# EnterpriseCV-6/Season-NeRF

Hardware: AMD Instinct MI355X
Metric: ray-samples/sec (4096 rays x 96 samples forward render, T_NeRF 8x256) (higher is better)
Workload: dtype i8x3 (16-bit fixed point as two int8 digits on v_mfma_i32_32x32x32_i8, exact int32 accumulate, fp32 epilogue)

## Files before the change

### include/season_nerf_hip.h

```cpp
#ifndef SEASON_NERF_HIP_H
#define SEASON_NERF_HIP_H

#include <stddef.h>
#include <stdint.h>

#ifdef __cplusplus
extern "C" {
#endif

#define SNERF_OK 0
#define SNERF_E_INVALID (-1)
#define SNERF_E_MISSING (-2)
#define SNERF_E_HIP (-3)
#define SNERF_E_STATE (-4)

typedef struct snerf_model snerf_model;

const char* snerf_last_error(void);
int snerf_abi_version(void);

snerf_model* snerf_model_create(int layer_width, int n_classes);
int snerf_model_set_tensor(snerf_model* m, const char* key, const float* host_data, size_t numel);
int snerf_model_finalize(snerf_model* m);
void snerf_model_destroy(snerf_model* m);
int snerf_model_width(const snerf_model* m);
int snerf_model_classes(const snerf_model* m);

#define SNERF_PREC_BF16X3 0
#define SNERF_PREC_BF16 1
#define SNERF_PREC_I8X3 2
#define SNERF_PREC_AUTO 3
int snerf_model_set_precision(snerf_model* m, int precision);
int snerf_model_precision(const snerf_model* m);

typedef struct snerf_i8_estimate {
    double head_rms[4];
    double hidden_rms;
    double worst;
    double rgb_pred;
    double budget;
    int64_t acc_bound;
    int ok;
} snerf_i8_estimate;
int snerf_model_i8_estimate(snerf_model* m, snerf_i8_estimate* out);
int snerf_model_resolve_precision(snerf_model* m);

int snerf_model_pack_host(snerf_model* m, int program, uint8_t* stream_out, size_t* stream_bytes,
                          float* bias_out, size_t* bias_floats);

int snerf_group_forward(const snerf_model* m, int64_t n_groups, const float* d_time, const float* d_sun,
                        float* d_classes, float* d_sky_raw, float* d_sky, void* stream);

typedef struct snerf_field_out {
    float* d_rho;
    float* d_solar_vis;
    float* d_col_raw;
    float* d_adjust;
    float* d_col;
    float* d_adjust_col;
    float* d_points;
} snerf_field_out;

int snerf_field_forward_points(const snerf_model* m, int variant, int64_t n_points, const float* d_points,
                               int64_t group_size, const float* d_sun, const float* d_classes,
                               const snerf_field_out* out, void* stream);

int snerf_field_forward_rays(const snerf_model* m, int variant, int64_t n_rays, int n_samples,
                             const float* d_top, const float* d_bot, const float* d_tvals,
                             int64_t rays_per_group, const float* d_sun, const float* d_classes,
                             const snerf_field_out* out, void* stream);

int snerf_field_ray_visibility(const snerf_model* m, int64_t n_rays, int n_samples, const float* d_top, const float* d_bot,
                               const float* d_tvals, int flags, float* d_vis, void* stream);

typedef struct snerf_composite_out {
    float* d_rgb;
    float* d_albedo;
    float* d_pv;
    float* d_pe;
    float* d_ps;
    float* d_delta;
    float* d_shadow;
    float* d_acc;
    float* d_surf_loc;
    float* d_surf_dist;
} snerf_composite_out;

int snerf_composite_rays(int64_t n_rays, int n_samples, const float* d_top, const float* d_bot, const float* d_tvals,
                         const float* d_rho, const float* d_col, const float* d_solar_vis, const float* d_sky,
                         int flags, const float* d_rho_prior, float trust,
                         const snerf_composite_out* out, void* stream);
int snerf_composite_rays_dt(int64_t n_rays, int n_samples, const float* d_top, const float* d_bot, const float* d_tvals,
                            const float* d_rho, const float* d_col, const float* d_solar_vis, const float* d_sky,
                            int flags, const float* d_rho_prior, const float* d_trust,
                            const snerf_composite_out* out, void* stream);

size_t snerf_render_workspace_bytes(int64_t n_rays, int n_samples, int n_classes);
int snerf_render_rays(const snerf_model* m, int64_t n_rays, int n_samples, const float* d_top, const float* d_bot,
                      const float* d_tvals, const float* d_sun, const float* d_time, int flags,
                      float* d_rgb, const snerf_field_out* field_out, const snerf_composite_out* comp_out,
                      void* d_workspace, size_t workspace_bytes, void* stream);

typedef struct snerf_sweep_out {
    float* d_season;
    float* d_shaded;
    float* d_base;
    float* d_shadow_adjust;
    float* d_raw_shadow;
    float* d_classic;
} snerf_sweep_out;

int snerf_composite_sweep(int64_t n_rays, int n_samples, int n_classes, int n_times, const float* d_top,
                          const float* d_bot, const float* d_tvals, const float* d_deltas, const float* d_rho, const float* d_col_raw,
                          const float* d_adjust, const float* d_solar_vis, const float* d_sky, const float* d_class_vecs,
                          int flags, const snerf_sweep_out* out, void* stream);

typedef struct snerf_trainer snerf_trainer;
snerf_trainer* snerf_trainer_create(int layer_width, int n_classes);
void snerf_trainer_destroy(snerf_trainer* t);
int snerf_trainer_classes(const snerf_trainer* t);
int64_t snerf_trainer_param_floats(const snerf_trainer* t);
int64_t snerf_trainer_buffer_floats(const snerf_trainer* t);
int snerf_trainer_tensor_count(const snerf_trainer* t);
int snerf_trainer_tensor_info(const snerf_trainer* t, int index, char* key, int key_cap, int* is_buffer, int64_t* offset,
                              int64_t* numel, int* rows, int* cols);
size_t snerf_trainer_workspace_bytes(snerf_trainer* t, int64_t n_rays, int64_t n_solar_rays, int n_samples);
int snerf_trainer_bind(snerf_trainer* t, float* d_params, float* d_grads, float* d_adam_m, float* d_adam_v, float* d_buffers,
                       void* d_workspace, size_t workspace_bytes, int64_t n_rays, int64_t n_solar_rays, int n_samples);
int snerf_trainer_bound_sizes(const snerf_trainer* t, int64_t* n_rays, int64_t* n_solar_rays, int* n_samples);
int snerf_trainer_forward_image(snerf_trainer* t, int64_t n_rays, int n_samples, const float* d_top, const float* d_bot,
                                const float* d_tvals, const float* d_sun, const float* d_time, int train_bn, int flags,
                                const snerf_composite_out* out, float* d_sky, float* d_classes,
                                const snerf_field_out* per_sample, void* stream);
int snerf_trainer_backward_image(snerf_trainer* t, const float* d_g_rgb, const float* d_g_albedo, const float* d_g_sky,
// ... 60 lines not shown
```

### season_nerf_amd/_lib.py

```python
import ctypes as C
import os

HERE = os.path.dirname(os.path.abspath(__file__))
LIB_PATH = os.environ.get("SNERF_LIB", os.path.join(HERE, "libseason_nerf_hip.so"))

_f = C.POINTER(C.c_float)


class FieldOut(C.Structure):
    _fields_ = [(n, C.c_void_p) for n in
                ("d_rho", "d_solar_vis", "d_col_raw", "d_adjust", "d_col", "d_adjust_col", "d_points")]


class CompositeOut(C.Structure):
    _fields_ = [(n, C.c_void_p) for n in
                ("d_rgb", "d_albedo", "d_pv", "d_pe", "d_ps", "d_delta", "d_shadow", "d_acc", "d_surf_loc", "d_surf_dist")]


class SweepOut(C.Structure):
    _fields_ = [(n, C.c_void_p) for n in ("d_season", "d_shaded", "d_base", "d_shadow_adjust", "d_raw_shadow", "d_classic")]


class I8Estimate(C.Structure):
    _fields_ = [("head_rms", C.c_double * 4), ("hidden_rms", C.c_double), ("worst", C.c_double),
                ("rgb_pred", C.c_double), ("budget", C.c_double), ("acc_bound", C.c_int64), ("ok", C.c_int)]


ALLREDUCE_FN = C.CFUNCTYPE(C.c_int, C.c_void_p, C.c_void_p, C.c_int64, C.c_int, C.c_void_p)

_lib = None


def lib():
    global _lib
    if _lib is not None:
        return _lib
    if not os.path.exists(LIB_PATH):
        raise RuntimeError(
            f"season_nerf_amd: HIP library not built ({LIB_PATH} missing). Run `python season_nerf_amd/build.py` "
            "(needs hipcc, gfx950). There is no CPU fallback.")
    L = C.CDLL(LIB_PATH)
    vp, i64, i32 = C.c_void_p, C.c_int64, C.c_int
    L.snerf_last_error.restype = C.c_char_p
    L.snerf_abi_version.restype = i32
    L.snerf_model_create.restype = vp
    L.snerf_model_create.argtypes = [i32, i32]
    L.snerf_model_set_tensor.argtypes = [vp, C.c_char_p, vp, C.c_size_t]
    L.snerf_model_finalize.argtypes = [vp]
    L.snerf_model_destroy.argtypes = [vp]
    L.snerf_model_destroy.restype = None
    L.snerf_model_width.argtypes = [vp]
    L.snerf_model_classes.argtypes = [vp]
    L.snerf_model_set_precision.argtypes = [vp, i32]
    L.snerf_model_precision.argtypes = [vp]
    L.snerf_model_i8_estimate.argtypes = [vp, C.POINTER(I8Estimate)]
    L.snerf_model_resolve_precision.argtypes = [vp]
    L.snerf_model_pack_host.argtypes = [vp, i32, vp, C.POINTER(C.c_size_t), vp, C.POINTER(C.c_size_t)]
    L.snerf_group_forward.argtypes = [vp, i64, vp, vp, vp, vp, vp, vp]
    L.snerf_field_forward_points.argtypes = [vp, i32, i64, vp, i64, vp, vp, C.POINTER(FieldOut), vp]
    L.snerf_field_forward_rays.argtypes = [vp, i32, i64, i32, vp, vp, vp, i64, vp, vp, C.POINTER(FieldOut), vp]
    L.snerf_field_ray_visibility.argtypes = [vp, i64, i32, vp, vp, vp, i32, vp, vp]
    L.snerf_composite_rays.argtypes = [i64, i32, vp, vp, vp, vp, vp, vp, vp, i32, vp, C.c_float,
                                       C.POINTER(CompositeOut), vp]
    L.snerf_composite_rays_dt.argtypes = [i64, i32, vp, vp, vp, vp, vp, vp, vp, i32, vp, vp, C.POINTER(CompositeOut), vp]
    L.snerf_render_workspace_bytes.restype = C.c_size_t
    L.snerf_render_workspace_bytes.argtypes = [i64, i32, i32]
    L.snerf_render_rays.argtypes = [vp, i64, i32, vp, vp, vp, vp, vp, i32, vp, C.POINTER(FieldOut),
                                    C.POINTER(CompositeOut), vp, C.c_size_t, vp]
    L.snerf_composite_sweep.argtypes = [i64, i32, i32, i32, vp, vp, vp, vp, vp, vp, vp, vp, vp, vp, i32, C.POINTER(SweepOut), vp]
    f32p = vp
    L.snerf_trainer_create.restype = vp
    L.snerf_trainer_create.argtypes = [i32, i32]
    L.snerf_trainer_destroy.argtypes = [vp]
    L.snerf_trainer_destroy.restype = None
    L.snerf_trainer_bound_sizes.restype = i32
    L.snerf_trainer_bound_sizes.argtypes = [vp, vp, vp, vp]
    L.snerf_trainer_classes.restype = i32
    L.snerf_trainer_classes.argtypes = [vp]
    L.snerf_trainer_param_floats.restype = i64
    L.snerf_trainer_param_floats.argtypes = [vp]
    L.snerf_trainer_buffer_floats.restype = i64
    L.snerf_trainer_buffer_floats.argtypes = [vp]
    L.snerf_trainer_tensor_count.argtypes = [vp]
    L.snerf_trainer_tensor_info.argtypes = [vp, i32, C.c_char_p, i32, C.POINTER(i32), C.POINTER(i64), C.POINTER(i64),
                                            C.POINTER(i32), C.POINTER(i32)]
    L.snerf_trainer_workspace_bytes.restype = C.c_size_t
    L.snerf_trainer_workspace_bytes.argtypes = [vp, i64, i64, i32]
    L.snerf_trainer_bind.argtypes = [vp, f32p, f32p, f32p, f32p, f32p, vp, C.c_size_t, i64, i64, i32]
    L.snerf_trainer_forward_image.argtypes = [vp, i64, i32, vp, vp, vp, vp, vp, i32, i32, C.POINTER(CompositeOut), vp, vp,
                                              C.POINTER(FieldOut), vp]
    L.snerf_trainer_backward_image.argtypes = [vp, vp, vp, vp, vp, vp, C.c_float, vp, vp, vp]
    L.snerf_trainer_backward_image_dt.argtypes = [vp, vp, vp, vp, vp, vp, vp, vp, vp, vp]
    L.snerf_trainer_backward_points.argtypes = [vp, vp, vp, vp, vp, vp, vp]
    L.snerf_trainer_forward_solar.argtypes = [vp, i64, i32, vp, vp, vp, vp, i32, vp, vp, vp, vp, vp, vp, vp, vp]
    L.snerf_trainer_backward_solar.argtypes = [vp, vp, vp]
    L.snerf_trainer_zero_grad.argtypes = [vp, vp]
    L.snerf_trainer_set_allreduce.argtypes = [vp, vp, vp, i32]
    L.snerf_trainer_debug_read.argtypes = [vp, C.c_char_p, vp, i64]
    L.snerf_trainer_adam_step.argtypes = [vp, C.c_float, C.c_float, C.c_float, C.c_float, i32, vp]
    L.snerf_trainer_adam_step_dev.argtypes = [vp, vp, vp]
    L.snerf_adam_step.argtypes = [vp, vp, vp, vp, i64, C.c_float, C.c_float, C.c_float, C.c_float, i32, vp]
    L.snerf_rays_from_camera.argtypes = [vp, i32, i32, i32, vp, vp, vp]
    L.snerf_ray_grid.argtypes = [i32, i32, i32, i64, i64, vp, i32, vp, vp, vp, vp, vp]
    L.snerf_prior_density.argtypes = [i64, vp, vp, vp, i32, i32, vp, vp, vp]
    L.snerf_surface_distance.argtypes = [i64, i32, vp, vp, vp, vp, i32, i32, vp, vp, vp]
    L.snerf_image_error.argtypes = [i64, vp, vp, vp, vp]
    L.snerf_transmittance.argtypes = [i64, i32, vp, vp, vp, vp]
    L.snerf_linear_scratch_bytes.restype = C.c_size_t
    L.snerf_linear_scratch_bytes.argtypes = [i32, i32]
    L.snerf_linear_forward.argtypes = [i64, i32, i32, vp, i64, vp, vp, C.c_float, vp, i64, vp, i32, vp, C.c_size_t, vp, i32, vp]
    L.snerf_linear_dgrad.argtypes = [i64, i32, i32, vp, i64, vp, i32, C.c_float, i32, vp, i64, i32, vp, C.c_size_t, vp, i64, vp, vp, vp, vp, vp]
    L.snerf_linear_wgrad.argtypes = [i64, i32, i32, vp, i64, vp, i64, C.c_float, vp, i32, vp, i32, vp]
    L.snerf_field_kernel_info.argtypes = [vp, i64, C.POINTER(i32), C.POINTER(i32), C.POINTER(i32)]
    _lib = L
    return L


PRECISIONS = {"bf16x3": 0, "bf16": 1, "i8x3": 2, "auto": 3}
PRECISION_NAMES = {0: "bf16x3", 1: "bf16", 2: "i8x3"}


def check(rc, what):
    if rc != 0:
        raise RuntimeError(f"season_nerf_amd: {what} failed (code {rc}): {lib().snerf_last_error().decode()}")


EXPORTS = ["snerf_last_error", "snerf_abi_version", "snerf_model_create", "snerf_model_set_tensor",
           "snerf_model_finalize", "snerf_model_destroy", "snerf_model_width", "snerf_model_classes",
           "snerf_model_set_precision", "snerf_model_precision", "snerf_model_i8_estimate", "snerf_model_resolve_precision",
           "snerf_model_pack_host", "snerf_group_forward", "snerf_field_forward_points", "snerf_field_forward_rays", "snerf_field_ray_visibility",
           "snerf_composite_rays", "snerf_composite_rays_dt", "snerf_composite_sweep", "snerf_render_workspace_bytes", "snerf_render_rays", "snerf_rays_from_camera", "snerf_ray_grid", "snerf_field_kernel_info",
           "snerf_prior_density", "snerf_surface_distance", "snerf_image_error", "snerf_transmittance",
           "snerf_linear_scratch_bytes", "snerf_linear_forward", "snerf_linear_dgrad", "snerf_linear_wgrad",
           "snerf_trainer_create", "snerf_trainer_destroy", "snerf_trainer_classes", "snerf_trainer_param_floats", "snerf_trainer_buffer_floats",
           "snerf_trainer_tensor_count", "snerf_trainer_tensor_info", "snerf_trainer_workspace_bytes", "snerf_trainer_bind", "snerf_trainer_bound_sizes",
           "snerf_trainer_forward_image", "snerf_trainer_backward_image", "snerf_trainer_backward_image_dt", "snerf_trainer_backward_points", "snerf_trainer_forward_solar",
           "snerf_trainer_backward_solar", "snerf_trainer_zero_grad", "snerf_trainer_set_allreduce", "snerf_trainer_adam_step", "snerf_trainer_adam_step_dev", "snerf_adam_step", "snerf_trainer_debug_read",
           "snerf_loss_scratch_bytes", "snerf_loss_scratch_init", "snerf_loss_terms_forward", "snerf_loss_terms_backward"]
```

### season_nerf_amd/build.py

```python
import os
import subprocess
import sys
from concurrent.futures import ThreadPoolExecutor

HERE = os.path.dirname(os.path.abspath(__file__))
REPO = os.path.dirname(HERE)
CSRC = os.path.join(HERE, "csrc")
OBJ = os.path.join(REPO, "build", "obj")
LIB = os.path.join(HERE, "libseason_nerf_hip.so")
SOURCES = ["kernels.hip", "kernels_i8.hip", "kernels_i8x2.hip", "kernels_i8_w512.hip", "kernels_ks.hip", "api.cpp", "pack.cpp", "gemm.hip", "gemm16.hip", "gemm_areg.hip", "train_kernels.hip", "train.cpp", "dsm.hip"]
HEADERS = ["gemm_common.h", "gemm_rows.h", "kernels.h", "linear_product.h", "mlp_device.h", "mlp_bf16_device.h", "mlp_i8_device.h", "pack.h", "program.h", "train.h", os.path.join("..", "..", "include", "season_nerf_hip.h")]
FLAGS = ["-std=c++17", "-O3", "--offload-arch=gfx950", "-fPIC", "-ffp-contract=off",
         "-mllvm", "-amdgpu-mfma-vgpr-form=1",
         "-Wno-unused-command-line-argument"]


EXTRA = {"kernels_i8_w512.hip": ["-mllvm", "-pragma-unroll-threshold=1000000"],
         "kernels_ks.hip": ["-mllvm", "-pragma-unroll-threshold=1000000"],
         "gemm_areg.hip": ["-mllvm", "-pragma-unroll-threshold=1000000"]}
INCLUDED = {"kernels_i8_w512.hip": ["kernels_i8.hip"]}


def _hipcc():
    return os.environ.get("HIPCC", "/opt/rocm/bin/hipcc")


def _newest_header():
    return max(os.path.getmtime(os.path.join(CSRC, h)) for h in HEADERS if os.path.exists(os.path.join(CSRC, h)))


def _obj(src):
    return os.path.join(OBJ, src + ".o")


def _deps(src):
    d = _obj(src) + ".d"
    if not os.path.exists(d):
        return None
    txt = open(d).read().replace("\\\n", " ")
    return [f for f in txt.split(":", 1)[1].split() if f.startswith(REPO)] if ":" in txt else None


def _stale(src, hdr_t):
    o = _obj(src)
    if not os.path.exists(o):
        return True
    t = os.path.getmtime(o)
    deps = _deps(src)
    if deps is not None:
        return any((not os.path.exists(f)) or os.path.getmtime(f) > t for f in deps)
    return any(os.path.getmtime(os.path.join(CSRC, f)) > t for f in [src] + INCLUDED.get(src, [])) or hdr_t > t


def needs_build():
    if not os.path.exists(LIB):
        return True
    hdr_t = _newest_header()
    t = os.path.getmtime(LIB)
    return any(os.path.getmtime(os.path.join(CSRC, s)) > t for s in SOURCES) or hdr_t > t


def _compile(src, verbose):
    cmd = [_hipcc()] + FLAGS + EXTRA.get(src, []) + ["-MD", "-MF", _obj(src) + ".d", "-c", os.path.join(CSRC, src), "-o", _obj(src)]
    if verbose:
        print(" ".join(cmd), flush=True)
    subprocess.check_call(cmd)


def build(force=False, verbose=True, jobs=None):
    if not force and not needs_build():
        return LIB
    os.makedirs(OBJ, exist_ok=True)
    hdr_t = _newest_header()
    todo = [s for s in SOURCES if force or _stale(s, hdr_t)]
    jobs = jobs or min(len(todo) or 1, max(1, (os.cpu_count() or 2) - 1), 6)
    with ThreadPoolExecutor(max_workers=jobs) as ex:
        list(ex.map(lambda s: _compile(s, verbose), todo))
    cmd = [_hipcc(), "--offload-arch=gfx950", "-shared", "-fPIC", "-o", LIB] + [_obj(s) for s in SOURCES]
    if verbose:
        print(" ".join(cmd), flush=True)
    subprocess.check_call(cmd)
    return LIB


OPS_LIB = os.path.join(HERE, "libseason_nerf_ops.so")
OPS_SRC = os.path.join(CSRC, "ops.cpp")


def build_ops(force=False, verbose=True):
    import torch
    if not force and os.path.exists(OPS_LIB) and os.path.getmtime(OPS_LIB) > max(os.path.getmtime(OPS_SRC), os.path.getmtime(LIB),
                                                                                  os.path.getmtime(os.path.join(REPO, "include", "season_nerf_hip.h"))):
        return OPS_LIB
# ... 18 lines not shown
```

### season_nerf_amd/csrc/api.cpp

```cpp
#include "../../include/season_nerf_hip.h"

#include <hip/hip_runtime.h>

#include <cstdio>
#include <cstdlib>
#include <cmath>
#include <cstring>
#include <string>

#include "kernels.h"
#include "pack.h"
#include "train.h"

#ifndef SNERF_I8_BUDGET
#define SNERF_I8_BUDGET 1.0e-4
#endif

using namespace snerf;

static thread_local std::string g_err;
static int fail(int code, const std::string& msg) {
    g_err = msg;
    return code;
}
int snerf_set_error(int code, const std::string& msg) { return fail(code, msg); }
static int fail_hip(hipError_t e, const char* what) {
    return fail(SNERF_E_HIP, std::string(what) + ": " + hipGetErrorString(e));
}

struct snerf_model {
    int W = 0, C = 0;
    int precision = SNERF_PREC_BF16X3;
    bool auto_mode = false;
    bool resolved = true;
    bool have_estimate = false;
    snerf_i8_estimate estimate{};
    Weights w;
    bool finalized = false;
    Packed host[2];
    Packed host_i8;
    Packed host_ks;
    Packed host_ksg;
    float* d_group_f32 = nullptr;
    size_t g32_off[10] = {0};
    uint8_t* d_stream[2] = {nullptr, nullptr};
    float* d_bias[2] = {nullptr, nullptr};
    uint8_t* d_stream_i8 = nullptr;
    float* d_table_i8 = nullptr;
    uint8_t* d_stream_ks = nullptr;
    float* d_bias_ks = nullptr;
    uint8_t* d_stream_ksg = nullptr;
    float* d_bias_ksg = nullptr;
    int n_cu = 0;
};

extern "C" {

const char* snerf_last_error(void) { return g_err.c_str(); }
int snerf_abi_version(void) { return 8; }

snerf_model* snerf_model_create(int layer_width, int n_classes) {
    if (layer_width != 64 && layer_width != 256 && layer_width != 512) {
        fail(SNERF_E_INVALID, "layer_width " + std::to_string(layer_width) +
                                  " has no compiled kernel (built widths: 64, 256, 512)");
        return nullptr;
    }
    if (n_classes < 1 || n_classes > kMaxClasses) {
        fail(SNERF_E_INVALID, "n_classes must be in [1," + std::to_string(kMaxClasses) + "]");
        return nullptr;
    }
    snerf_model* m = new snerf_model();
    m->W = layer_width;
    m->C = n_classes;
    return m;
}

int snerf_model_set_precision(snerf_model* m, int precision) {
    if (!m) return fail(SNERF_E_INVALID, "NULL model");
    if (m->finalized) return fail(SNERF_E_STATE, "model already finalized (set the precision before snerf_model_finalize)");
    if (precision != SNERF_PREC_BF16X3 && precision != SNERF_PREC_BF16 && precision != SNERF_PREC_I8X3 && precision != SNERF_PREC_AUTO)
        return fail(SNERF_E_INVALID, "unknown precision mode " + std::to_string(precision));
    m->auto_mode = precision == SNERF_PREC_AUTO;
    m->resolved = !m->auto_mode;
    m->precision = precision;
    return SNERF_OK;
}
// ... 173 lines not shown
                m->g32_off[2 * i + j] = blob.size();
                blob.insert(blob.end(), t->data.begin(), t->data.end());
                blob.resize((blob.size() + 3) / 4 * 4, 0.f);
            }
        const int W = m->W, C = m->C, W4 = W / 4;
        const size_t want[10] = {(size_t)W * 10, (size_t)W, (size_t)W * W, (size_t)W, (size_t)C * W, (size_t)C, (size_t)W4 * 27, (size_t)W4, (size_t)3 * W4, 3};
        for (int i = 0; i < 10; ++i) {
            const size_t have = (i < 9 ? m->g32_off[i + 1] : blob.size()) - m->g32_off[i];
            if (have < want[i] || have >= want[i] + 4) return fail(SNERF_E_INVALID, std::string("tensor of ") + keys[i / 2] + " has the wrong size");
        }
        if ((e = hipMalloc((void**)&m->d_group_f32, blob.size() * 4)) != hipSuccess) return fail_hip(e, "hipMalloc");
        if ((e = hipMemcpy(m->d_group_f32, blob.data(), blob.size() * 4, hipMemcpyHostToDevice)) != hipSuccess) return fail_hip(e, "hipMemcpy");
    }
    m->finalized = true;
    return SNERF_OK;
}

void snerf_model_destroy(snerf_model* m) {
    if (!m) return;
    for (int p = 0; p < 2; ++p) {
        if (m->d_stream[p]) (void)hipFree(m->d_stream[p]);
        if (m->d_bias[p]) (void)hipFree(m->d_bias[p]);
    }
    if (m->d_stream_i8) (void)hipFree(m->d_stream_i8);
    if (m->d_table_i8) (void)hipFree(m->d_table_i8);
    if (m->d_stream_ks) (void)hipFree(m->d_stream_ks);
    if (m->d_bias_ks) (void)hipFree(m->d_bias_ks);
    if (m->d_stream_ksg) (void)hipFree(m->d_stream_ksg);
    if (m->d_bias_ksg) (void)hipFree(m->d_bias_ksg);
    if (m->d_group_f32) (void)hipFree(m->d_group_f32);
    delete m;
}

int snerf_model_width(const snerf_model* m) { return m ? m->W : 0; }
int snerf_model_classes(const snerf_model* m) { return m ? m->C : 0; }

static int check_ready(const snerf_model* m) {
    if (!m) return fail(SNERF_E_INVALID, "NULL model");
    if (!m->finalized) return fail(SNERF_E_STATE, "model not finalized (call snerf_model_finalize)");
    return SNERF_OK;
}

static int group_forward_f32(const snerf_model* m, int64_t R, const float* d_time, const float* d_sun, float* d_classes, float* d_sky_raw,
                             float* d_sky, hipStream_t st) {
    const int W = m->W, C = m->C, W4 = W / 4;
    const size_t per_ray = 12 + (size_t)2 * W + 8 + 28 + W4 + 4;
    float* ws = nullptr;
    hipError_t e = hipMallocAsync((void**)&ws, per_ray * (size_t)R * 4, st);
    if (e != hipSuccess) return fail_hip(e, "hipMallocAsync (per-ray network scratch)");
    float *pe_t = ws, *h1 = pe_t + 12 * R, *h2 = h1 + (size_t)W * R, *logits = h2 + (size_t)W * R, *pe_s = logits + 8 * R, *k1 = pe_s + 28 * R,
          *sky_raw = k1 + (size_t)W4 * R;
    const float* P = m->d_group_f32;
    auto linear = [&](int layer, const float* in, int64_t ld_in, int K, float* out, int64_t ld_out, int N, float alpha) {
        GemmArgs g{};
        g.A = in; g.B = P + m->g32_off[2 * layer]; g.C = out;
        g.M = R; g.N = N; g.K = K;
        g.sAm = ld_in; g.sAk = 1; g.sBk = 1; g.sBn = K; g.ldc = ld_out;
        g.alpha = alpha; g.bias = P + m->g32_off[2 * layer + 1]; g.colsum = nullptr; g.flags = 0; g.splitk = 1;
        return launch_gemm(g, st);
    };
#define GF(x) do { if ((e = (x)) != hipSuccess) { (void)hipFreeAsync(ws, st); return fail_hip(e, "per-ray network (fp32)"); } } while (0)
    if (d_classes) {
        GF(launch_pe_small(d_time, 4, 2, PE_TIME_N, R, pe_t, 12, st));
        GF(linear(0, pe_t, 12, PE_TIME_F, h1, W, W, 30.f));
        GF(launch_sin_fwd(h1, h1, R, W, W, W, nullptr, nullptr, nullptr, nullptr, st));
        GF(linear(1, h1, W, W, h2, W, W, 30.f));
        GF(launch_sin_fwd(h2, h2, R, W, W, W, nullptr, nullptr, nullptr, nullptr, st));
        GF(linear(2, h2, W, W, logits, C, C, 1.f));
        GF(launch_softmax(logits, d_classes, R, C, st));
    }
    if (d_sky_raw || d_sky) {
        float* raw = d_sky_raw ? d_sky_raw : sky_raw;
        GF(launch_pe_small(d_sun, 3, 3, PE_SUN_N, R, pe_s, 28, st));
        GF(linear(3, pe_s, 28, PE_SUN_F, k1, W4, W4, 30.f));
        GF(launch_sin_fwd(k1, k1, R, W4, W4, W4, nullptr, nullptr, nullptr, nullptr, st));
        GF(linear(4, k1, W4, W4, raw, 3, 3, 1.f));
        if (d_sky) GF(launch_sigmoid(raw, d_sky, R * 3, st));
    }
#undef GF
    e = hipFreeAsync(ws, st);
    return e == hipSuccess ? SNERF_OK : fail_hip(e, "hipFreeAsync");
}

int snerf_group_forward(const snerf_model* m, int64_t n_groups, const float* d_time, const float* d_sun,
                        float* d_classes, float* d_sky_raw, float* d_sky, void* stream) {
    int rc = check_ready(m);
    if (rc) return rc;
    if (n_groups == 0) return SNERF_OK;
    if (n_groups < 0 || !d_time || !d_sun) return fail(SNERF_E_INVALID, "snerf_group_forward: bad argument");
    static const bool group_f32 = getenv("SNERF_GROUP_F32") != nullptr;
    if (m->d_group_f32 && (group_f32 || !m->d_stream_ksg)) return group_forward_f32(m, n_groups, d_time, d_sun, d_classes, d_sky_raw, d_sky, (hipStream_t)stream);
    MlpArgs a{};
    const bool ks = ks_width(m->W);
    a.stream = ks ? m->d_stream_ksg : m->d_stream[PROG_GROUP];
    a.stream_bytes = ks ? (uint32_t)group_chunks_ks(m->W, m->C) * kChunkBytes : (uint32_t)m->host[PROG_GROUP].stream.size();
    a.bias = ks ? m->d_bias_ksg : m->d_bias[PROG_GROUP];
    a.bias_floats = (int)m->host[PROG_GROUP].bias.size();
    a.n = n_groups;
    a.n_classes = m->C;
    a.group_size = 1;
    a.time = d_time;
    a.sun = d_sun;
    a.g_classes = d_classes;
    a.g_sky_raw = d_sky_raw;
    a.g_sky = d_sky;
    hipError_t e = ks ? launch_mlp_ks_group(m->W, a, m->n_cu, (hipStream_t)stream)
                      : launch_mlp(PROG_GROUP, m->W, 0, false, a, m->n_cu, (hipStream_t)stream);
    return e == hipSuccess ? SNERF_OK : fail_hip(e, "group kernel launch");
}

static int field_launch(const snerf_model* m, int variant, MlpArgs& a, const snerf_field_out* out, void* stream) {
    if (variant < 0 || variant > 3 || (variant == 3 && !(a.out.vis && a.top && a.bot && a.tvals && !a.points)))
        return fail(SNERF_E_INVALID, "variant must be 0, 1 or 2 (3, ray visibility, only through snerf_field_ray_visibility)");
    if (variant == 3 && m->precision == SNERF_PREC_BF16) return fail(SNERF_E_INVALID, "ray visibility: not available in the bf16 fast mode");
    a.stream = m->d_stream[PROG_FIELD];
    a.stream_bytes = (uint32_t)field_variant_chunks(m->W, m->C, variant) * kChunkBytes;
    a.bias = m->d_bias[PROG_FIELD];
    a.bias_floats = (int)m->host[PROG_FIELD].bias.size();
    a.n_classes = m->C;
#ifdef SNERF_ABLATE
    if (const char* e = getenv("SNERF_ABLATE")) a.debug = (uint32_t)atoi(e);
#endif
    if (out) {
        a.out.rho = out->d_rho; a.out.solar_vis = out->d_solar_vis; a.out.col_raw = out->d_col_raw;
        a.out.adjust = out->d_adjust; a.out.col = out->d_col; a.out.adjust_col = out->d_adjust_col;
        a.out.points = out->d_points;
    }
    if (variant <= 1 && !a.sun) return fail(SNERF_E_INVALID, "sun directions are required for variants 0 and 1");
    hipError_t e;
    if (m->precision == SNERF_PREC_I8X3) {
        a.stream = m->d_stream_i8;
        a.stream_bytes = (uint32_t)field_variant_chunks_i8(m->W, m->C, variant) * kChunkBytes;
        a.bias = m->d_table_i8;
        a.bias_floats = (int)m->host_i8.bias.size();
        static const bool one_wave = getenv("SNERF_I8_ONE_WAVE") != nullptr;
        if (m->W <= 256 && !one_wave) e = launch_mlp_i8x2(m->W, variant, a, m->n_cu, (hipStream_t)stream);
        else e = launch_mlp_i8(m->W, variant, a, m->n_cu, (hipStream_t)stream);
    } else if (ks_width(m->W)) {
        a.stream = m->d_stream_ks;
        a.stream_bytes = (uint32_t)field_variant_chunks_ks(m->W, m->C, variant) * kChunkBytes;
        a.bias = m->d_bias_ks;
        a.bias_floats = (int)m->host_ks.bias.size();
        e = launch_mlp_ks(m->W, variant, a, m->n_cu, (hipStream_t)stream);
    } else {
        e = launch_mlp(PROG_FIELD, m->W, variant, m->precision == SNERF_PREC_BF16, a, m->n_cu, (hipStream_t)stream);
    }
    return e == hipSuccess ? SNERF_OK : fail_hip(e, "field kernel launch");
}

int snerf_field_forward_points(const snerf_model* m, int variant, int64_t n_points, const float* d_points,
                               int64_t group_size, const float* d_sun, const float* d_classes,
                               const snerf_field_out* out, void* stream) {
    int rc = check_ready(m);
    if (rc) return rc;
    if (n_points == 0) return SNERF_OK;
    if (n_points < 0 || !d_points || group_size < 1) return fail(SNERF_E_INVALID, "snerf_field_forward_points: bad argument");
    MlpArgs a{};
    a.n = n_points;
    a.points = d_points;
    a.n_samples = 1;
    a.group_size = group_size;
    a.sun = d_sun;
    a.classes = d_classes;
    return field_launch(m, variant, a, out, stream);
}

int snerf_field_forward_rays(const snerf_model* m, int variant, int64_t n_rays, int n_samples, const float* d_top,
                             const float* d_bot, const float* d_tvals, int64_t rays_per_group, const float* d_sun,
                             const float* d_classes, const snerf_field_out* out, void* stream) {
    int rc = check_ready(m);
    if (rc) return rc;
    if (n_rays == 0) return SNERF_OK;
    if (n_rays < 0 || n_samples < 1 || rays_per_group < 1 || !d_top || !d_bot || !d_tvals)
        return fail(SNERF_E_INVALID, "snerf_field_forward_rays: bad argument");
    MlpArgs a{};
    a.n = n_rays * n_samples;
    a.top = d_top;
    a.bot = d_bot;
    a.tvals = d_tvals;
    a.n_samples = n_samples;
    a.group_size = (int64_t)n_samples * rays_per_group;
    a.sun = d_sun;
    a.classes = d_classes;
    return field_launch(m, variant, a, out, stream);
}

int snerf_field_ray_visibility(const snerf_model* m, int64_t n_rays, int n_samples, const float* d_top, const float* d_bot,
                               const float* d_tvals, int flags, float* d_vis, void* stream) {
    int rc = check_ready(m);
// ... 201 lines not shown
```

### season_nerf_amd/csrc/kernels.h

```cpp
#pragma once
#include <hip/hip_runtime.h>
#include <stdint.h>

namespace snerf {

struct snerf_field_out_dev {
    float* rho;
    float* solar_vis;
    float* col_raw;
    float* adjust;
    float* col;
    float* adjust_col;
    float* points;
    float* vis;
};

constexpr int kVoteBytes = 64;

struct MlpArgs {
    const uint8_t* stream;
    uint32_t stream_bytes;
    const float* bias;
    int bias_floats;
    int64_t n;
    int n_classes;
    const float* points;
    const float* top;
    const float* bot;
    const float* tvals;
    int n_samples;
    int64_t group_size;
    const float* sun;
    const float* classes;
    snerf_field_out_dev out;
    const float* time;
    float* g_classes;
    float* g_sky_raw;
    float* g_sky;
    uint32_t debug;
    int ray_flags;
};

struct CompOutDev {
    float *rgb, *albedo, *pv, *pe, *ps, *delta, *shadow, *acc, *surf_loc, *surf_dist;
};

struct CompArgs {
    int64_t n_rays;
    int n_samples;
    const float *top, *bot, *tvals;
    const float *rho, *col, *solar_vis, *sky;
    int flags;
    const float* rho_prior;
    float trust;
    const float* trust_dev;
    CompOutDev out;
};

struct RayGenArgs {
    double P[12];
    int rows, cols, ds;
    float* rows_out;
    uint8_t* valid;
};
hipError_t launch_rays_from_camera(const RayGenArgs& a, hipStream_t st);

struct RayGridArgs {
    int mode;
    int rows, cols;
    int64_t lo, hi;
    double q[3];
    int has_region;
    double region[4];
    double P[12];
    int img_rows, img_cols;
    float *top, *bot;
    uint8_t* valid;
    int32_t* pix;
};
hipError_t launch_ray_grid(const RayGridArgs& a, hipStream_t st);

struct SweepArgs {
    int64_t n_rays;
    int n_samples, n_classes, n_times, flags;
    const float *top, *bot, *tvals;
    const float* deltas;
    const float *rho, *col_raw, *adjust, *solar_vis;
    int adjust_vec4;
    const float* sky;
    const float* class_vecs;
    float *season, *shaded;
    float* classic;
    float *base, *shadow_adjust, *raw_shadow;
};
hipError_t launch_sweep(const SweepArgs& a, hipStream_t st);
__host__ __device__ inline int64_t field_tiles(int64_t n, int variant, int pts, int rays) { return variant == 3 ? (n + rays - 1) / rays : (n + pts - 1) / pts; }
hipError_t launch_fused(void (*kernel)(MlpArgs), int64_t n_tiles, int block, int lds_bytes, const MlpArgs& a, int n_cu, hipStream_t st);
hipError_t launch_mlp(int prog, int W, int variant, bool fast, const MlpArgs& a, int n_cu, hipStream_t st);
hipError_t launch_mlp_i8(int W, int variant, const MlpArgs& a, int n_cu, hipStream_t st);
int field_variant_chunks_i8(int W, int C, int variant);
hipError_t launch_mlp_i8x2(int W, int variant, const MlpArgs& a, int n_cu, hipStream_t st);
hipError_t launch_mlp_ks(int W, int variant, const MlpArgs& a, int n_cu, hipStream_t st);
hipError_t launch_mlp_ks_group(int W, const MlpArgs& a, int n_cu, hipStream_t st);
int field_variant_chunks_ks(int W, int C, int variant);
int group_chunks_ks(int W, int C);
int mlp_ks_lds_bytes(int bias_floats);
int mlp_ks_tile_points();
hipError_t launch_composite(const CompArgs& a, hipStream_t st);
hipError_t launch_prior_density(int64_t n, const float* pts, const float* delta, const double* hm, int hx, int hy, const float* outside,
                                float neg_log_term, float* rho, hipStream_t st);
hipError_t launch_surface_distance(int64_t n_rays, int S, const float* top, const float* bot, const float* tvals, const double* dsm, int dx,
                                   int dy, const double* levels, double* dist, hipStream_t st);
hipError_t launch_image_error(int64_t n_pix, const float* img, const float* gt, double* sums, hipStream_t st);
hipError_t launch_transmittance(int64_t n_rays, int S, const float* rho, const float* delta, float* pv, hipStream_t st);
int mlp_lds_bytes(int bias_floats);
int mlp_tile_points();
int field_variant_chunks(int W, int C, int variant);
const char* mlp_kernel_name();

}
```

Measured before the change: 520.9 million.

## Add split-wave group MLP kernel spreading time layers and heads across waves

Adds a new group-level kernel that splits the time-embedding MLP output blocks across four waves, exchanging activations through LDS, then runs the class head and sun/sky head on separate waves with prefetched weight rings. It becomes the default for the non-ks group path, replacing the single-wave generic program, with an env/API switch to revert. This is meant to cut the latency of the per-group MLP, at the cost of extra LDS traffic and syncthreads. The measured ray-render workload may touch this group kernel only lightly, if at all.

```diff
diff --git a/include/season_nerf_hip.h b/include/season_nerf_hip.h
--- a/include/season_nerf_hip.h
+++ b/include/season_nerf_hip.h
@@ -50,6 +50,7 @@
 
 int snerf_group_forward(const snerf_model* m, int64_t n_groups, const float* d_time, const float* d_sun,
                         float* d_classes, float* d_sky_raw, float* d_sky, void* stream);
+int snerf_set_group_kernel(int mode);
 
 typedef struct snerf_field_out {
     float* d_rho;
diff --git a/season_nerf_amd/_lib.py b/season_nerf_amd/_lib.py
--- a/season_nerf_amd/_lib.py
+++ b/season_nerf_amd/_lib.py
@@ -57,6 +57,7 @@
     L.snerf_model_resolve_precision.argtypes = [vp]
     L.snerf_model_pack_host.argtypes = [vp, i32, vp, C.POINTER(C.c_size_t), vp, C.POINTER(C.c_size_t)]
     L.snerf_group_forward.argtypes = [vp, i64, vp, vp, vp, vp, vp, vp]
+    L.snerf_set_group_kernel.argtypes = [i32]
     L.snerf_field_forward_points.argtypes = [vp, i32, i64, vp, i64, vp, vp, C.POINTER(FieldOut), vp]
     L.snerf_field_forward_rays.argtypes = [vp, i32, i64, i32, vp, vp, vp, i64, vp, vp, C.POINTER(FieldOut), vp]
     L.snerf_field_ray_visibility.argtypes = [vp, i64, i32, vp, vp, vp, i32, vp, vp]
@@ -128,7 +129,7 @@
 EXPORTS = ["snerf_last_error", "snerf_abi_version", "snerf_model_create", "snerf_model_set_tensor",
            "snerf_model_finalize", "snerf_model_destroy", "snerf_model_width", "snerf_model_classes",
            "snerf_model_set_precision", "snerf_model_precision", "snerf_model_i8_estimate", "snerf_model_resolve_precision",
-           "snerf_model_pack_host", "snerf_group_forward", "snerf_field_forward_points", "snerf_field_forward_rays", "snerf_field_ray_visibility",
+           "snerf_model_pack_host", "snerf_group_forward", "snerf_set_group_kernel", "snerf_field_forward_points", "snerf_field_forward_rays", "snerf_field_ray_visibility",
            "snerf_composite_rays", "snerf_composite_rays_dt", "snerf_composite_sweep", "snerf_render_workspace_bytes", "snerf_render_rays", "snerf_rays_from_camera", "snerf_ray_grid", "snerf_field_kernel_info",
            "snerf_prior_density", "snerf_surface_distance", "snerf_image_error", "snerf_transmittance",
            "snerf_linear_scratch_bytes", "snerf_linear_forward", "snerf_linear_dgrad", "snerf_linear_wgrad",
diff --git a/season_nerf_amd/build.py b/season_nerf_amd/build.py
--- a/season_nerf_amd/build.py
+++ b/season_nerf_amd/build.py
@@ -8,7 +8,7 @@
 CSRC = os.path.join(HERE, "csrc")
 OBJ = os.path.join(REPO, "build", "obj")
 LIB = os.path.join(HERE, "libseason_nerf_hip.so")
-SOURCES = ["kernels.hip", "kernels_i8.hip", "kernels_i8x2.hip", "kernels_i8_w512.hip", "kernels_ks.hip", "api.cpp", "pack.cpp", "gemm.hip", "gemm16.hip", "gemm_areg.hip", "train_kernels.hip", "train.cpp", "dsm.hip"]
+SOURCES = ["kernels.hip", "kernels_i8.hip", "kernels_i8x2.hip", "kernels_i8_w512.hip", "kernels_ks.hip", "kernels_group.hip", "api.cpp", "pack.cpp", "gemm.hip", "gemm16.hip", "gemm_areg.hip", "train_kernels.hip", "train.cpp", "dsm.hip"]
 HEADERS = ["gemm_common.h", "gemm_rows.h", "kernels.h", "linear_product.h", "mlp_device.h", "mlp_bf16_device.h", "mlp_i8_device.h", "pack.h", "program.h", "train.h", os.path.join("..", "..", "include", "season_nerf_hip.h")]
 FLAGS = ["-std=c++17", "-O3", "--offload-arch=gfx950", "-fPIC", "-ffp-contract=off",
          "-mllvm", "-amdgpu-mfma-vgpr-form=1",
diff --git a/season_nerf_amd/csrc/api.cpp b/season_nerf_amd/csrc/api.cpp
--- a/season_nerf_amd/csrc/api.cpp
+++ b/season_nerf_amd/csrc/api.cpp
@@ -2,6 +2,7 @@
 
 #include <hip/hip_runtime.h>
 
+#include <atomic>
 #include <cstdio>
 #include <cstdlib>
 #include <cmath>
@@ -341,6 +342,16 @@
     return e == hipSuccess ? SNERF_OK : fail_hip(e, "hipFreeAsync");
 }
 
+static std::atomic<int>& group_kernel_mode() {
+    static std::atomic<int> mode{getenv("SNERF_GROUP_ONE_WAVE") != nullptr ? 1 : 0};
+    return mode;
+}
+int snerf_set_group_kernel(int mode) {
+    if (mode != 0 && mode != 1) return fail(SNERF_E_INVALID, "snerf_set_group_kernel: mode must be 0 (split) or 1 (one wave)");
+    group_kernel_mode().store(mode);
+    return SNERF_OK;
+}
+
 int snerf_group_forward(const snerf_model* m, int64_t n_groups, const float* d_time, const float* d_sun,
                         float* d_classes, float* d_sky_raw, float* d_sky, void* stream) {
     int rc = check_ready(m);
@@ -364,6 +375,7 @@
     a.g_sky_raw = d_sky_raw;
     a.g_sky = d_sky;
     hipError_t e = ks ? launch_mlp_ks_group(m->W, a, m->n_cu, (hipStream_t)stream)
+                : group_kernel_mode().load() == 0 ? launch_mlp_group_split(m->W, a, m->n_cu, (hipStream_t)stream)
                       : launch_mlp(PROG_GROUP, m->W, 0, false, a, m->n_cu, (hipStream_t)stream);
     return e == hipSuccess ? SNERF_OK : fail_hip(e, "group kernel launch");
 }
diff --git a/season_nerf_amd/csrc/kernels.h b/season_nerf_amd/csrc/kernels.h
--- a/season_nerf_amd/csrc/kernels.h
+++ b/season_nerf_amd/csrc/kernels.h
@@ -102,6 +102,7 @@
 hipError_t launch_mlp_i8x2(int W, int variant, const MlpArgs& a, int n_cu, hipStream_t st);
 hipError_t launch_mlp_ks(int W, int variant, const MlpArgs& a, int n_cu, hipStream_t st);
 hipError_t launch_mlp_ks_group(int W, const MlpArgs& a, int n_cu, hipStream_t st);
+hipError_t launch_mlp_group_split(int W, const MlpArgs& a, int n_cu, hipStream_t st);
 int field_variant_chunks_ks(int W, int C, int variant);
 int group_chunks_ks(int W, int C);
 int mlp_ks_lds_bytes(int bias_floats);
diff --git a/season_nerf_amd/csrc/kernels_group.hip b/season_nerf_amd/csrc/kernels_group.hip
--- /dev/null
+++ b/season_nerf_amd/csrc/kernels_group.hip
@@ -0,0 +1,222 @@
+#include "mlp_bf16_device.h"
+
+namespace snerf {
+
+constexpr int GS_TILE = 32;
+constexpr int GS_PF = 8;
+
+typedef __attribute__((address_space(3))) u32x4 lds_u32x4;
+
+typedef __amdgpu_buffer_rsrc_t Rsrc;
+__device__ __forceinline__ Rsrc make_rsrc(const void* p, uint32_t bytes) {
+    return __builtin_amdgcn_make_buffer_rsrc(const_cast<void*>(p), 0, (int)bytes, 0x00020000);
+}
+__device__ __forceinline__ u32x4 load16(Rsrc r, uint32_t voff, uint32_t soff) {
+    return __builtin_bit_cast(u32x4, __builtin_amdgcn_raw_buffer_load_b128(r, (int)voff, (int)soff, 0));
+}
+
+__host__ __device__ constexpr int ring_depth(int np) { return np < GS_PF ? np : GS_PF; }
+template <int N>
+__device__ __forceinline__ void request_weights(Rsrc wr, uint32_t base, uint32_t voff, u32x4* hi, u32x4* lo) {
+#pragma unroll
+    for (int q = 0; q < N; ++q) {
+        hi[q] = load16(wr, voff, base + q * kPairBytes);
+        lo[q] = load16(wr, voff, base + q * kPairBytes + kFragBytes);
+    }
+}
+__device__ __forceinline__ f32x16 request_bias(Rsrc br, int start, int b, uint32_t hoff) {
+    f32x16 acc;
+#pragma unroll
+    for (int q = 0; q < 4; ++q) {
+        const f32x4 t = __builtin_bit_cast(f32x4, load16(br, hoff, (start + b * 32) * 4 + q * 16));
+        acc[4 * q] = t[0]; acc[4 * q + 1] = t[1]; acc[4 * q + 2] = t[2]; acc[4 * q + 3] = t[3];
+    }
+    return acc;
+}
+
+template <int NBW, int KS, bool SIN>
+__device__ __forceinline__ void run_blocks(Rsrc wr, uint32_t base, uint32_t voff, u32x4* whi, u32x4* wlo, const f32x16* init, const Frag* in, Frag* out, f32x16* raw) {
+    constexpr int NP = NBW * KS, D = ring_depth(NP);
+    constexpr bool PIPE = KS >= 4;
+    f32x16 accs[2];
+    EpiTmp et[8];
+#pragma unroll
+    for (int b = 0; b < NBW; ++b) {
+        f32x16 acc = init[b];
+#pragma unroll
+        for (int s = 0; s < KS; ++s) {
+            const int q = b * KS + s;
+            const u32x4 a_hi = whi[q % D], a_lo = wlo[q % D];
+            if (q + D < NP) {
+                whi[q % D] = load16(wr, voff, base + (q + D) * kPairBytes);
+                wlo[q % D] = load16(wr, voff, base + (q + D) * kPairBytes + kFragBytes);
+            }
+            acc = mfma3(a_hi, a_lo, in[s], acc);
+            if (SIN && b > 0) {
+#pragma unroll
+                for (int e = 0; e < 8; ++e) {
+                    if (PIPE) {
+                        const int sA = 1 + (e * (KS - 4)) / 8;
+                        if (s == sA + 2) epi_C(e, et[e], out + 2 * (b - 1));
+                        if (s == sA + 1) epi_B(e, et[e], out + 2 * (b - 1));
+                        if (s == sA) epi_A(accs[(b - 1) & 1], e, et[e]);
+                    } else if (s == 0) {
+                        epi_A(accs[(b - 1) & 1], e, et[e]);
+                        epi_B(e, et[e], out + 2 * (b - 1));
+                        epi_C(e, et[e], out + 2 * (b - 1));
+                    }
+                }
+            }
+            __builtin_amdgcn_sched_barrier(0);
+        }
+        accs[b & 1] = acc;
+    }
+    if constexpr (SIN) {
+#pragma unroll
+        for (int e = 0; e < 8; ++e) epi_A(accs[(NBW - 1) & 1], e, et[e]);
+#pragma unroll
+        for (int e = 0; e < 8; ++e) epi_B(e, et[e], out + 2 * (NBW - 1));
+#pragma unroll
+        for (int e = 0; e < 8; ++e) epi_C(e, et[e], out + 2 * (NBW - 1));
+    } else {
+        *raw = accs[0];
+    }
+}
+
+template <int NBW>
+__device__ __forceinline__ void store_act(lds_char* buf, int b0, int lane, const Frag* out) {
+#pragma unroll
+    for (int f = 0; f < 2 * NBW; ++f) {
+        lds_char* p = buf + (2 * b0 + f) * kPairBytes + lane * 16;
+        *(lds_u32x4*)p = out[f].hi;
+        *(lds_u32x4*)(p + kFragBytes) = out[f].lo;
+    }
+}
+template <int KS>
+__device__ __forceinline__ void load_act(lds_char* buf, int lane, Frag* in) {
+#pragma unroll
+    for (int s = 0; s < KS; ++s) {
+        lds_char* p = buf + s * kPairBytes + lane * 16;
+        in[s].hi = *(lds_cu32x4*)p;
+        in[s].lo = *(lds_cu32x4*)(p + kFragBytes);
+    }
+}
+
+template <int W>
+__global__ __launch_bounds__(256, 1) void mlp_group_split_kernel(const MlpArgs A) {
+    extern __shared__ __attribute__((aligned(16))) char smem[];
+    constexpr int C_MAX = kMaxClasses;
+    constexpr int KW = W / 16, NB = W / 32, W4P = pad32(W / 4), KW4 = W4P / 16, NB4 = W4P / 32;
+    constexpr int BPW = NB >= 4 ? NB / 4 : 1;
+    constexpr int NWV = NB / BPW;
+    constexpr int ACT_BYTES = KW * kPairBytes;
+    lds_char* buf0 = (lds_char*)smem;
+    lds_char* buf1 = buf0 + ACT_BYTES;
+
+    const int lane = threadIdx.x & 63;
+    const int wave = __builtin_amdgcn_readfirstlane(threadIdx.x >> 6);
+    const int h = lane >> 5;
+    const int C = A.n_classes;
+    const bool owner = NWV == 4 || wave < NWV;
+    const int b0 = owner ? wave * BPW : 0;
+    const bool cls = wave == 0;
+    const uint32_t voff = lane * 16, hoff = h * 64;
+
+#define W_AT(L) (uint32_t)(prog_chunk_start(PROG_GROUP, W, C_MAX, L) * kChunkBytes)
+#define B_AT(L) prog_bias_start(PROG_GROUP, W, C_MAX, L)
+    const Rsrc wr = make_rsrc(A.stream, A.stream_bytes), br = make_rsrc(A.bias, (uint32_t)A.bias_floats * 4);
+    constexpr uint32_t w_t1 = W_AT(G_T1), w_t2 = W_AT(G_T2), w_cl = W_AT(G_CL), w_k1 = W_AT(G_K1), w_k2 = W_AT(G_K2);
+    const uint32_t voff_t1 = voff + b0 * PETIME_KS * kPairBytes, voff_t2 = voff + b0 * KW * kPairBytes;
+
+    const int64_t n_tiles = (A.n + GS_TILE - 1) / GS_TILE;
+    for (int64_t tile = blockIdx.x; tile < n_tiles; tile += gridDim.x) {
+        const int64_t n = tile * GS_TILE + (lane & 31);
+        const bool valid = n < A.n;
+        const int64_t nc = valid ? n : A.n - 1;
+
+        const float t0 = A.time[nc * 4], t1 = A.time[nc * 4 + 1];
+        const float s0 = A.sun[nc * 3], s1 = A.sun[nc * 3 + 1], s2 = A.sun[nc * 3 + 2];
+        constexpr int D1 = ring_depth(BPW * PETIME_KS), D2 = ring_depth(BPW * KW);
+        u32x4 w1h[D1], w1l[D1], w2h[D2], w2l[D2];
+        f32x16 it1[BPW], it2[BPW];
+        request_weights<D1>(wr, w_t1, voff_t1, w1h, w1l);
+        request_weights<D2>(wr, w_t2, voff_t2, w2h, w2l);
+#pragma unroll
+        for (int i = 0; i < BPW; ++i) {
+            it1[i] = request_bias(br, B_AT(G_T1), i, hoff + b0 * 128);
+            it2[i] = request_bias(br, B_AT(G_T2), i, hoff + b0 * 128);
+        }
+        __builtin_amdgcn_sched_barrier(0);
+
+        if (owner) {
+            Frag pt[PETIME_KS];
+            make_pe_time(t0, t1, h, pt);
+            Frag o[2 * BPW];
+            run_blocks<BPW, PETIME_KS, true>(wr, w_t1, voff_t1, w1h, w1l, it1, pt, o, nullptr);
+            store_act<BPW>(buf0, b0, lane, o);
+        }
+        __syncthreads();
+        if (owner) {
+            Frag in[KW];
+            load_act<KW>(buf0, lane, in);
+            Frag o[2 * BPW];
+            run_blocks<BPW, KW, true>(wr, w_t2, voff_t2, w2h, w2l, it2, in, o, nullptr);
+            store_act<BPW>(buf1, b0, lane, o);
+        }
+        constexpr int DH = ring_depth(KW), NK1 = NB4 * PESUN_KS;
+        static_assert(NK1 + KW4 <= DH, "the sun branch's pairs must fit the class head's ring");
+        u32x4 hh[DH], hl[DH];
+        f32x16 ih[NB4 + 1];
+        const uint32_t voff_h1 = voff + (cls ? w_cl : w_k1), voff_h2 = voff + (cls ? w_cl : w_k2 - NK1 * kPairBytes);
+        request_weights<NK1>(wr, 0, voff_h1, hh, hl);
+        request_weights<DH - NK1>(wr, NK1 * kPairBytes, voff_h2, hh + NK1, hl + NK1);
+        static_assert(B_AT(G_K2) == B_AT(G_K1) + 32 * NB4, "G_K2's biases follow G_K1's");
+#pragma unroll
+        for (int i = 0; i <= NB4; ++i) ih[i] = request_bias(br, 0, i, hoff + 4 * (cls ? B_AT(G_CL) : B_AT(G_K1)));
+        __builtin_amdgcn_sched_barrier(0);
+        __syncthreads();
+        if (cls) {
+            Frag in[KW];
+            load_act<KW>(buf1, lane, in);
+            f32x16 raw;
+            run_blocks<1, KW, false>(wr, w_cl, voff, hh, hl, ih, in, nullptr, &raw);
+            if (h == 0 && valid) {
+                float m = -3.0e38f;
+#pragma unroll
+                for (int c = 0; c < C_MAX; ++c) if (c < C) m = fmaxf(m, raw[c]);
+                float e[C_MAX], sum = 0.f;
+#pragma unroll
+                for (int c = 0; c < C_MAX; ++c) { e[c] = c < C ? expf(raw[c] - m) : 0.f; sum += e[c]; }
+#pragma unroll
+                for (int c = 0; c < C_MAX; ++c) if (c < C && A.g_classes) A.g_classes[n * C + c] = e[c] / sum;
+            }
+        } else if (wave == 1) {
+            Frag ps[PESUN_KS];
+            make_pe_sun(s0, s1, s2, h, ps);
+            Frag kA[KW4];
+            f32x16 raw;
+            run_blocks<NB4, PESUN_KS, true>(wr, w_k1, voff, hh, hl, ih, ps, kA, nullptr);
+            run_blocks<1, KW4, false>(wr, w_k2, voff, hh + NK1, hl + NK1, ih + NB4, kA, nullptr, &raw);
+            if (h == 0 && valid) {
+#pragma unroll
+                for (int k = 0; k < 3; ++k) {
+                    if (A.g_sky_raw) A.g_sky_raw[n * 3 + k] = raw[k];
+                    if (A.g_sky) A.g_sky[n * 3 + k] = sigmoid_f(raw[k]);
+                }
+            }
+        }
+    }
+#undef W_AT
+#undef B_AT
+}
+
+int mlp_group_split_lds_bytes(int W) { return 2 * (W / 16) * kPairBytes; }
+
+hipError_t launch_mlp_group_split(int W, const MlpArgs& a, int n_cu, hipStream_t st) {
+    const int64_t n_tiles = (a.n + GS_TILE - 1) / GS_TILE;
+    if (W == 64) return launch_fused(mlp_group_split_kernel<64>, n_tiles, 256, mlp_group_split_lds_bytes(64), a, n_cu, st);
+    if (W == 256) return launch_fused(mlp_group_split_kernel<256>, n_tiles, 256, mlp_group_split_lds_bytes(256), a, n_cu, st);
+    return hipErrorInvalidValue;
+}
+
+}
```

Result: faster. 526.7 million (median of 6 runs) (+1.1%).
